# SoyeonHH/MMDA

Hardware: AMD Instinct MI355X
Metric: training samples/sec on MOSEI-shaped synthetic batch (higher is better)
Workload: dtype bf16; 1 GPU; MISA train step, MOSEI shapes B=32/GPU T=50 (d_t,d_v,d_a)=(300,35,74) hidden=128 V=20000, bf16 MFMA operands fp32 accumulate, dropout on, full lengths; global_batch=32, seq_len=50, parallelism=single, use_confidNet=False, rnncell=lstm, dp_global_stats=False

## Files before the change

### mmda_amd/csrc/fused_rows.h

```cpp
#pragma once
#include "../../include/mmda_hip.h"
#include <stdint.h>

struct FusedBwdC {
  int B, hs, ncls, nb;
  const float* tcp; const float* scores; const float* d_tcp; const float* d_scores; float* d_logits;
  float p_cls; uint64_t seed; int site_cls;
  const float* head_w;
  float* d_hfused;
  mmda_ln_bwd_args ln2;
  float* pg_parts;
  const float* d_recon; const float* rec_wT; float* rec_part;
};

struct FusedBwdA {
  int B, hs, nhead, nb;
  mmda_ln_bwd_args ln1;
  const float* ffn_parts; int n_parts; float* d_x1;
  const float* d_attn_out; const float* out_wT; float* d_ctx;
  const float* qkv; const float* probs; float* d_qkv; float p_tf; uint64_t seed; int site_attn;
  const float* in_wT;
  const float* d_recon;
  const float* rec_part;
  const float* rec_wT;
  const float* x6;
  float* d_x6;
  const float* priv_wT;
  const float* sh_wT;
  float* d_orig;
  mmda_ln_bwd_args lnp[3];
  float* pg_parts;
  unsigned long long* dbg;
  const unsigned* wait_flag; unsigned wait_value; unsigned* wait_err;
};

struct FusedFwdA {
  int B, hs, nhead, nb;
  const float* x6;
  const float* rec_w; const float* rec_b; float* recon;
  const float* in_w; const float* in_b; float* qkv;
  float* ctx; float* probs; float p_tf; uint64_t seed; int site_attn;
  const float* out_w; const float* out_b; float* attn_out;
  mmda_ln_args ln1;
  const float* orig; float* d_recon; float* d_orig; float recon_inv_n, recon_scale;
  int split_recon;
};
struct FusedFwdC {
  int B, hs, ncls, nb;
  mmda_ln_args ln2;
  const float* ffn_parts; int n_parts; const float* b2; float* f2;
  const float* hfused; const float* head_w; const float* head_b; float* logits;
  float threshold; float* tcp; float* scores; float* labels; float p_cls; uint64_t seed; int site_cls;
  const float* emo; float* d_scores;
};
struct FusedFfnFwd {
  int M, hs, F, S;
  const float* x1; const float* w1; const float* b1; float* f1;
  float p; uint64_t seed; int site;
  const float* w2;
  float* parts;
};
struct FusedFfnBwd {
  int M, hs, F, S;
  const float* d_f2; const float* f1; float gate_scale;
  const float* l2_wT;
  float* d_f1;
  const float* l1_wT;
  float* parts;
};
int mmda_fused_ffn_fwd(const FusedFfnFwd* a, void* stream);
int mmda_fused_ffn_bwd(const FusedFfnBwd* a, void* stream);
int mmda_fused_fwd_a(const FusedFwdA* a, void* stream);
int mmda_fused_fwd_c(const FusedFwdC* a, void* stream);
int mmda_fused_bwd_c(const FusedBwdC* a, void* stream);
int mmda_fused_bwd_a(const FusedBwdA* a, void* stream);
constexpr int FUSED_PG_SLOTS = 5;
int mmda_fused_pg_finish(const float* pg_parts, int B, int hs, float* const* dgamma, float* const* dbeta, void* stream);
extern "C" int mmda_debug_set_fused_stamps(void* device_buffer);
```

### mmda_amd/csrc/fused_rows.hip

```cpp
#include "common.h"
#include "rowlocal.h"
#include "fused_rows.h"

namespace {

typedef __attribute__((ext_vector_type(4))) float f4;
constexpr int FR_THREADS = 512;

struct MacRound { f4 a[8], b[8]; };
constexpr int WL_LD = 128 + 4;
struct WRows { f4 g[8]; };
__device__ __forceinline__ void wrows_load(WRows& W, const float* __restrict__ bblk, int ldb, int lane) {
#pragma unroll
  for (int j = 0; j < 8; ++j) W.g[j] = *reinterpret_cast<const f4*>(bblk + (int64_t)(2 * j + (lane >> 5)) * ldb + 4 * (lane & 31));
}
__device__ __forceinline__ void wrows_to_lds(const WRows& W, float* wl, int lane) {
#pragma unroll
  for (int j = 0; j < 8; ++j) *reinterpret_cast<f4*>(wl + (2 * j + (lane >> 5)) * WL_LD + 4 * (lane & 31)) = W.g[j];
}
__device__ __forceinline__ void mac_frags(MacRound& R, const float* arow , const float* wl, int lane) {
  const int r16 = lane & 15, g = lane >> 4;
  const f4 z = {0.f, 0.f, 0.f, 0.f};
#pragma unroll
  for (int c = 0; c < 8; ++c) {
    R.a[c] = arow ? *reinterpret_cast<const f4*>(arow + 16 * c + 4 * g) : z;
    R.b[c] = *reinterpret_cast<const f4*>(wl + r16 * WL_LD + 16 * c + 4 * g);
  }
}
__device__ __forceinline__ void mac_run(f32x4& acc, const MacRound& R) {
#pragma unroll
  for (int c = 0; c < 8; ++c)
#pragma unroll
    for (int s = 0; s < 4; ++s) acc = __builtin_amdgcn_mfma_f32_16x16x4f32(R.a[c][s], R.b[c][s], acc, 0, 0, 0);
}
template <int NR>
__device__ __forceinline__ void tile_mac_chain(f32x4& acc, const float* const (&ar)[NR], const float* const (&bblk)[NR], const int (&ldb)[NR],
                                               int lane, float* wl ) {
  WRows W;
  MacRound R;
  wrows_load(W, bblk[0], ldb[0], lane);
#pragma unroll
  for (int r = 0; r < NR; ++r) {
    wrows_to_lds(W, wl, lane);
    if (r + 1 < NR) wrows_load(W, bblk[r + 1], ldb[r + 1], lane);
    mac_frags(R, ar[r], wl, lane);
    mac_run(acc, R);
  }
}

__device__ __forceinline__ float sum_parts(const float* __restrict__ p, int n, int64_t stride) {
  float acc = 0.f;
  int q = 0;
  for (; q + 16 <= n; q += 16) {
    float v[16];
#pragma unroll
    for (int u = 0; u < 16; ++u) v[u] = p[(q + u) * stride];
#pragma unroll
    for (int u = 0; u < 16; ++u) acc += v[u];
  }
  for (; q < n; ++q) acc += p[q * stride];
  return acc;
}

template <typename RowOff, typename Finish>
__device__ __forceinline__ void sum_parts_rows(const float* __restrict__ parts, int n, int64_t stride, int groups, RowOff row_off, f4* lds,
                                               Finish finish) {
  const int n0 = (n + 1) >> 1;
  for (int it = threadIdx.x; it < 2 * groups; it += FR_THREADS) {
    const int gi = it % groups, half = it / groups;
    const float* p = parts + row_off(gi) + (int64_t)(half ? n0 : 0) * stride;
    const int cnt = half ? n - n0 : n0;
    f4 acc = {0.f, 0.f, 0.f, 0.f};
    int q = 0;
    for (; q + 16 <= cnt; q += 16) {
      f4 v[16];
#pragma unroll
      for (int u = 0; u < 16; ++u) v[u] = *reinterpret_cast<const f4*>(p + (q + u) * stride);
#pragma unroll
      for (int u = 0; u < 16; ++u) acc += v[u];
    }
    for (; q < cnt; ++q) acc += *reinterpret_cast<const f4*>(p + q * stride);
    lds[half * groups + gi] = acc;
  }
  __syncthreads();
  for (int gi = threadIdx.x; gi < groups; gi += FR_THREADS) finish(gi, lds[gi] + lds[groups + gi]);
  __syncthreads();
}

__device__ __forceinline__ void stage_sync() {
  __threadfence_block();
  __syncthreads();
}

constexpr int LDS_A_FLOATS = 12 * (384 + 4) + 18 * (128 + 4);
template <typename SrcOf>
__device__ __forceinline__ void stage_rows(float* lds, int nrows, int K, SrcOf src_of) {
  const int per_row = K >> 2;
  for (int e = threadIdx.x; e < nrows * per_row; e += FR_THREADS) {
    const int r = e / per_row, c = e % per_row;
    const float* src = src_of(r);
    const f4 z = {0.f, 0.f, 0.f, 0.f};
    *reinterpret_cast<f4*>(lds + r * (K + 4) + 4 * c) = src ? *reinterpret_cast<const f4*>(src + 4 * c) : z;
  }
  __syncthreads();
}

template <typename RowOf>
__device__ __forceinline__ void ln_bwd_rows(const mmda_ln_bwd_args& a, int nrows, RowOf row_of, float* red ,
                                            float* part) {
  const int lane = threadIdx.x & 63, wave = threadIdx.x >> 6;
  float dg[2] = {0.f, 0.f}, db[2] = {0.f, 0.f};
  for (int i = wave; i < nrows; i += FR_THREADS / 64) ln_bwd_row<2>(a, row_of(i), lane, dg, db);
  if (part == nullptr) return;
#pragma unroll
  for (int q = 0; q < 2; ++q) { red[(0 * 8 + wave) * 128 + q * 64 + lane] = dg[q]; red[(1 * 8 + wave) * 128 + q * 64 + lane] = db[q]; }
  __syncthreads();
  for (int i = threadIdx.x; i < 128; i += FR_THREADS) {
    float gsum = 0.f, bsum = 0.f;
#pragma unroll
    for (int w = 0; w < 8; ++w) { gsum += red[(0 * 8 + w) * 128 + i]; bsum += red[(1 * 8 + w) * 128 + i]; }
    part[i] = i < a.n ? gsum : 0.f;
    part[128 + i] = i < a.n ? bsum : 0.f;
  }
  __syncthreads();
}
__device__ __forceinline__ float* pg_slot(float* parts, int b, int k) { return parts ? parts + ((int64_t)b * FUSED_PG_SLOTS + k) * 256 : nullptr; }
__device__ __forceinline__ void pg_zero_rest(float* parts, int b0, int nb, int k) {
  if (!parts) return;
  for (int e = threadIdx.x; e < (nb - 1) * 256; e += FR_THREADS) pg_slot(parts, b0 + 1 + e / 256, k)[e % 256] = 0.f;
}

__device__ __forceinline__ void rec_part_rows(const FusedBwdC& P, int b0, int nb, float* lds_a, float* lds_w) {
  const int B = P.B, hs = P.hs;
  const int lane = threadIdx.x & 63, wave = threadIdx.x >> 6;
  const int r16 = lane & 15, g = lane >> 4;
  const int nmod = 3 * nb;
  const bool mok = r16 < nmod;
  const int mi = mok ? r16 / nb : 0;
  const int col = wave * 16 + r16;
  stage_rows(lds_a, nmod, hs, [&](int r) { return P.d_recon + ((int64_t)(r / nb) * B + b0 + (r % nb)) * hs; });
  f32x4 acc = {0.f, 0.f, 0.f, 0.f};
  const float* row = mok ? lds_a + r16 * (hs + 4) : nullptr;
  const float* const ar[3] = {(mok && mi == 0) ? row : nullptr, (mok && mi == 1) ? row : nullptr, (mok && mi == 2) ? row : nullptr};
  const float* rw = P.rec_wT + (int64_t)wave * 16 * hs;
  const float* const bb[3] = {rw, rw + (int64_t)hs * hs, rw + (int64_t)2 * hs * hs};
  const int ld[3] = {hs, hs, hs};
  tile_mac_chain<3>(acc, ar, bb, ld, lane, lds_w + wave * 16 * WL_LD);
#pragma unroll
  for (int i = 0; i < 4; ++i) {
    const int r = 4 * g + i;
    if (r < nmod) P.rec_part[((int64_t)(r / nb) * B + b0 + (r % nb)) * hs + col] = acc[i];
  }
}

__global__ __launch_bounds__(FR_THREADS) void fused_bwd_c_kernel(FusedBwdC P) {
  __shared__ float red[2 * 8 * 128];
  __shared__ __attribute__((aligned(16))) float lds_a[6 * (128 + 4)];
  __shared__ __attribute__((aligned(16))) float lds_w[8 * 16 * WL_LD];
  const int nblk = (P.B + P.nb - 1) / P.nb;
  if ((int)blockIdx.x >= nblk) {
    const int rb0 = ((int)blockIdx.x - nblk) * P.nb;
    rec_part_rows(P, rb0, min(P.nb, P.B - rb0), lds_a, lds_w);
    return;
  }
  const int b0 = (int)blockIdx.x * P.nb;
  const int nb = min(P.nb, P.B - b0);
  const int NC = 6 + P.ncls, B = P.B, hs = P.hs;
  for (int e = threadIdx.x; e < nb * NC; e += FR_THREADS) {
    const int b = b0 + e / NC, c = e % NC;
    float g = 0.f;
    if (c < 6) {
      if (P.d_tcp) { const float t = P.tcp[b * 6 + c]; g = P.d_tcp[b * 6 + c] * t * (1.f - t); }
    } else {
      const int k = c - 6;
      if (P.d_scores) {
        const float s = P.scores[b * P.ncls + k];
        g = P.d_scores[b * P.ncls + k] * s * (1.f - s) * drop_mul(P.p_cls, P.seed, P.site_cls, (uint64_t)(b * P.ncls + k));
      }
    }
    P.d_logits[b * NC + c] = g;
  }
  stage_sync();
  const int W6 = 6 * hs;
  for (int e = threadIdx.x; e < nb * W6; e += FR_THREADS) {
    const int b = b0 + e / W6, n = e % W6;
    float acc = 0.f;
    for (int c = 0; c < NC; ++c) acc += P.d_logits[b * NC + c] * P.head_w[(int64_t)c * W6 + n];
    P.d_hfused[(int64_t)b * W6 + n] = acc;
  }
  stage_sync();
  ln_bwd_rows(P.ln2, S6K * nb, [&](int i) { return (i / nb) * B + b0 + (i % nb); }, red, pg_slot(P.pg_parts, b0, 0));
  pg_zero_rest(P.pg_parts, b0, nb, 0);
}

__global__ __launch_bounds__(FR_THREADS) void fused_bwd_a_kernel(FusedBwdA P) {
  __shared__ float red[2 * 8 * 128];
  __shared__ __attribute__((aligned(16))) float lds_a[LDS_A_FLOATS];
  __shared__ __attribute__((aligned(16))) float lds_w[8 * 16 * WL_LD];
  const int b0 = (int)blockIdx.x * P.nb;
  const int nb = min(P.nb, P.B - b0);
  const int B = P.B, hs = P.hs;
  const int lane = threadIdx.x & 63, wave = threadIdx.x >> 6;
  const int r16 = lane & 15, g = lane >> 4;
  const int64_t BH = (int64_t)B * hs;
  int stamp_i = 0;
  auto stamp = [&]() { if (P.dbg && blockIdx.x == 0 && threadIdx.x == 0) P.dbg[stamp_i] = __builtin_readcyclecounter(); ++stamp_i; };
  stamp();
  flag_wait(P.wait_flag, P.wait_value, P.wait_err);
  if (P.ffn_parts) {
    const int64_t MH = (int64_t)S6K * B * hs;
    auto off = [&](int gi) { const int i = gi / (hs / 4); return ((int64_t)(i / nb) * B + b0 + (i % nb)) * hs + 4 * (gi % (hs / 4)); };
    sum_parts_rows(P.ffn_parts, P.n_parts, MH, S6K * nb * (hs / 4), off, reinterpret_cast<f4*>(lds_a), [&](int gi, f4 t) {
      f4* d = reinterpret_cast<f4*>(P.d_x1 + off(gi));
      *d = *d + t;
    });
    stage_sync();
  }
  ln_bwd_rows(P.ln1, S6K * nb, [&](int i) { return (i / nb) * B + b0 + (i % nb); }, red, pg_slot(P.pg_parts, b0, 1));
  pg_zero_rest(P.pg_parts, b0, nb, 1);
  stage_sync();
  stamp();
  const int ntok = S6K * nb;
  const bool rok = r16 < ntok;
  const int tj = rok ? r16 / nb : 0;
  const int col = wave * 16 + r16;
  {
    f32x4 acc = {0.f, 0.f, 0.f, 0.f};
    stage_rows(lds_a, ntok, hs, [&](int r) { return P.d_attn_out + ((int64_t)(r / nb) * B + b0 + (r % nb)) * hs; });
    const float* const ar[1] = {rok ? lds_a + r16 * (hs + 4) : nullptr};
    const float* const bb[1] = {P.out_wT + (int64_t)wave * 16 * hs};
    const int ld[1] = {hs};
    tile_mac_chain<1>(acc, ar, bb, ld, lane, lds_w + wave * 16 * WL_LD);
#pragma unroll
    for (int i = 0; i < 4; ++i) {
      const int r = 4 * g + i;
      if (r < ntok) P.d_ctx[((int64_t)(r / nb) * B + b0 + (r % nb)) * hs + col] = acc[i];
    }
  }
  stage_sync();
  stamp();
  for (int pr = wave; pr < nb * P.nhead; pr += FR_THREADS / 64)
    attn_bwd_hd64_one(P.qkv, P.probs, P.d_ctx, B, P.d_qkv, P.p_tf, P.seed, P.site_attn, P.nhead, (b0 + pr / P.nhead) * P.nhead + pr % P.nhead, lane);
  stage_sync();
  stamp();
  {
    f32x4 acc = {0.f, 0.f, 0.f, 0.f};
    float* lds_r = lds_a + 12 * (3 * hs + 4);
    stage_rows(lds_a, ntok, 3 * hs, [&](int r) { return P.d_qkv + ((int64_t)(r / nb) * B + b0 + (r % nb)) * 3 * hs; });
    const float* qrow = rok ? lds_a + r16 * (3 * hs + 4) : nullptr;
    const float* wrow = P.in_wT + (int64_t)wave * 16 * 3 * hs;
    if (P.rec_part) {
      const float* const ar[3] = {qrow, qrow ? qrow + 128 : nullptr, qrow ? qrow + 256 : nullptr};
      const float* const bb[3] = {wrow, wrow + 128, wrow + 256};
      const int ld[3] = {3 * hs, 3 * hs, 3 * hs};
      tile_mac_chain<3>(acc, ar, bb, ld, lane, lds_w + wave * 16 * WL_LD);
    } else {
      stage_rows(lds_r, ntok, hs, [&](int r) { return P.d_recon + ((int64_t)((r / nb) % 3) * B + b0 + (r % nb)) * hs; });
      const float* rec_row = rok ? lds_r + r16 * (hs + 4) : nullptr;
      const float* const ar[6] = {qrow, qrow ? qrow + 128 : nullptr, qrow ? qrow + 256 : nullptr, (rok && tj % 3 == 0) ? rec_row : nullptr,
                                  (rok && tj % 3 == 1) ? rec_row : nullptr, (rok && tj % 3 == 2) ? rec_row : nullptr};
      const float* recw = P.rec_wT + (int64_t)wave * 16 * hs;
      const float* const bb[6] = {wrow, wrow + 128, wrow + 256, recw, recw + (int64_t)hs * hs, recw + (int64_t)2 * hs * hs};
      const int ld[6] = {3 * hs, 3 * hs, 3 * hs, hs, hs, hs};
      tile_mac_chain<6>(acc, ar, bb, ld, lane, lds_w + wave * 16 * WL_LD);
    }
#pragma unroll
    for (int i = 0; i < 4; ++i) {
      const int r = 4 * g + i;
      if (r < ntok) {
        const int64_t o = ((int64_t)(r / nb) * B + b0 + (r % nb)) * hs + col;
        const float s = P.x6[o];
        float t = acc[i];
        if (P.rec_part) t += P.rec_part[((int64_t)((r / nb) % 3) * B + b0 + (r % nb)) * hs + col];
        P.d_x6[o] = (P.d_x6[o] + t) * (s * (1.f - s));
      }
    }
  }
  stage_sync();
  stamp();
  const int nmod = 3 * nb;
  const bool mok = r16 < nmod;
  const int mi = mok ? r16 / nb : 0;
  {
    f32x4 acc = {0.f, 0.f, 0.f, 0.f};
    stage_rows(lds_a, 2 * nmod, hs, [&](int r) { return P.d_x6 + ((int64_t)((r / nmod) * 3 + (r % nmod) / nb) * B + b0 + (r % nb)) * hs; });
    const float* prow = mok ? lds_a + r16 * (hs + 4) : nullptr;
    const float* const ar[4] = {mok ? lds_a + (nmod + r16) * (hs + 4) : nullptr, (mok && mi == 0) ? prow : nullptr,
                                (mok && mi == 1) ? prow : nullptr, (mok && mi == 2) ? prow : nullptr};
    const float* pw = P.priv_wT + (int64_t)wave * 16 * hs;
    const float* const bb[4] = {P.sh_wT + (int64_t)wave * 16 * hs, pw, pw + (int64_t)hs * hs, pw + (int64_t)2 * hs * hs};
    const int ld[4] = {hs, hs, hs, hs};
    tile_mac_chain<4>(acc, ar, bb, ld, lane, lds_w + wave * 16 * WL_LD);
#pragma unroll
    for (int i = 0; i < 4; ++i) {
      const int r = 4 * g + i;
      if (r < nmod) {
        const int64_t o = ((int64_t)(r / nb) * B + b0 + (r % nb)) * hs + col;
        P.d_orig[o] += acc[i];
      }
    }
  }
  stage_sync();
  stamp();
  for (int i = wave; i < 3 * nb; i += FR_THREADS / 64) {
    const mmda_ln_bwd_args& a = P.lnp[i / nb];
    float dg[2] = {0.f, 0.f}, db[2] = {0.f, 0.f};
    ln_bwd_row<2>(a, b0 + i % nb, lane, dg, db);
    float* part = pg_slot(P.pg_parts, b0 + i % nb, 2 + i / nb);
    if (part) {
#pragma unroll
      for (int q = 0; q < 2; ++q) {
        const int c = q * 64 + lane;
        part[c] = c < a.n ? dg[q] : 0.f;
        part[128 + c] = c < a.n ? db[q] : 0.f;
      }
    }
  }
  (void)BH;
  stamp();
}

__global__ __launch_bounds__(FR_THREADS) void fused_fwd_a_kernel(FusedFwdA P) {
  __shared__ __attribute__((aligned(16))) float lds_a[LDS_A_FLOATS];
  __shared__ __attribute__((aligned(16))) float lds_w[8 * 16 * WL_LD];
  const int nblk = (P.B + P.nb - 1) / P.nb;
  const bool do_recon = !P.split_recon || (int)blockIdx.x >= nblk;
  const bool do_chain = !P.split_recon || (int)blockIdx.x < nblk;
  const int b0 = ((int)blockIdx.x % nblk) * P.nb;
  const int nb = min(P.nb, P.B - b0);
  const int B = P.B, hs = P.hs;
  const int lane = threadIdx.x & 63, wave = threadIdx.x >> 6;
  const int r16 = lane & 15, g = lane >> 4;
  const int ntok = S6K * nb, nmod = 3 * nb;
  const bool rok = r16 < ntok;
  const bool mok = r16 < nmod;
  const int mi = mok ? r16 / nb : 0;
  const int col = wave * 16 + r16;
  stage_rows(lds_a, ntok, hs, [&](int r) { return P.x6 + ((int64_t)(r / nb) * B + b0 + (r % nb)) * hs; });
  if (do_recon) {
  for (int e = threadIdx.x; e < nmod * (hs / 4); e += FR_THREADS) {
    const int r = e / (hs / 4), c = e % (hs / 4);
    const f4 a = *reinterpret_cast<const f4*>(lds_a + r * (hs + 4) + 4 * c), b2 = *reinterpret_cast<const f4*>(lds_a + (nmod + r) * (hs + 4) + 4 * c);
    *reinterpret_cast<f4*>(lds_a + (12 + r) * (hs + 4) + 4 * c) = a + b2;
  }
  __syncthreads();
  {
    f32x4 acc = {0.f, 0.f, 0.f, 0.f};
    const float* srow = mok ? lds_a + (12 + r16) * (hs + 4) : nullptr;
    const float* const ar[3] = {(mok && mi == 0) ? srow : nullptr, (mok && mi == 1) ? srow : nullptr, (mok && mi == 2) ? srow : nullptr};
    const float* rw = P.rec_w + (int64_t)wave * 16 * hs;
    const float* const bb[3] = {rw, rw + (int64_t)hs * hs, rw + (int64_t)2 * hs * hs};
    const int ld[3] = {hs, hs, hs};
    tile_mac_chain<3>(acc, ar, bb, ld, lane, lds_w + wave * 16 * WL_LD);
#pragma unroll
    for (int i = 0; i < 4; ++i) {
      const int r = 4 * g + i;
      if (r < nmod) {
        const int64_t o = ((int64_t)(r / nb) * B + b0 + (r % nb)) * hs + col;
        const float rv = acc[i] + P.rec_b[(r / nb) * hs + col];
        P.recon[o] = rv;
        if (P.d_recon) {
          const float d = rv - P.orig[o];
          const float gr = 2.f * d * P.recon_inv_n * P.recon_scale;
          P.d_recon[o] = gr;
          P.d_orig[o] = 0.f - gr;
        }
      }
    }
  }
  }
  if (!do_chain) return;
#pragma unroll 1
  for (int pass = 0; pass < 3; ++pass) {
    const int n = pass * 128 + col;
    f32x4 acc = {0.f, 0.f, 0.f, 0.f};
    const float* const ar[1] = {rok ? lds_a + r16 * (hs + 4) : nullptr};
    const float* const bb[1] = {P.in_w + (int64_t)(pass * 128 + wave * 16) * hs};
    const int ld[1] = {hs};
    tile_mac_chain<1>(acc, ar, bb, ld, lane, lds_w + wave * 16 * WL_LD);
    const float bias = P.in_b[n];
#pragma unroll
    for (int i = 0; i < 4; ++i) {
      const int r = 4 * g + i;
      if (r < ntok) P.qkv[((int64_t)(r / nb) * B + b0 + (r % nb)) * 3 * hs + n] = acc[i] + bias;
    }
  }
  stage_sync();
  for (int pr = wave; pr < nb * P.nhead; pr += FR_THREADS / 64)
    attn_fwd_hd64_one(P.qkv, B, P.ctx, P.probs, P.p_tf, P.seed, P.site_attn, P.nhead, (b0 + pr / P.nhead) * P.nhead + pr % P.nhead, lane);
  stage_sync();
  {
    f32x4 acc = {0.f, 0.f, 0.f, 0.f};
    stage_rows(lds_a, ntok, hs, [&](int r) { return P.ctx + ((int64_t)(r / nb) * B + b0 + (r % nb)) * hs; });
    const float* const ar[1] = {rok ? lds_a + r16 * (hs + 4) : nullptr};
    const float* const bb[1] = {P.out_w + (int64_t)wave * 16 * hs};
    const int ld[1] = {hs};
    tile_mac_chain<1>(acc, ar, bb, ld, lane, lds_w + wave * 16 * WL_LD);
    const float bias = P.out_b[col];
#pragma unroll
    for (int i = 0; i < 4; ++i) {
      const int r = 4 * g + i;
      if (r < ntok) P.attn_out[((int64_t)(r / nb) * B + b0 + (r % nb)) * hs + col] = acc[i] + bias;
    }
  }
  stage_sync();
  for (int i = wave; i < ntok; i += FR_THREADS / 64) ln_fwd_row<2>(P.ln1, (i / nb) * B + b0 + (i % nb), lane);
}

__global__ __launch_bounds__(FR_THREADS) void fused_fwd_c_kernel(FusedFwdC P) {
  __shared__ f4 sp[2 * 12 * 32];
  const int b0 = (int)blockIdx.x * P.nb;
  const int nb = min(P.nb, P.B - b0);
  const int B = P.B, hs = P.hs, NC = 6 + P.ncls, W6 = 6 * hs;
  const int lane = threadIdx.x & 63, wave = threadIdx.x >> 6;
  if (P.ffn_parts) {
    const int64_t MH = (int64_t)S6K * B * hs;
    auto off = [&](int gi) { const int i = gi / (hs / 4); return ((int64_t)(i / nb) * B + b0 + (i % nb)) * hs + 4 * (gi % (hs / 4)); };
    sum_parts_rows(P.ffn_parts, P.n_parts, MH, S6K * nb * (hs / 4), off, sp, [&](int gi, f4 t) {
      const float* b = P.b2 + 4 * (gi % (hs / 4));
      *reinterpret_cast<f4*>(P.f2 + off(gi)) = t + f4{b[0], b[1], b[2], b[3]};
    });
    stage_sync();
  }
  for (int i = wave; i < S6K * nb; i += FR_THREADS / 64) ln_fwd_row<2>(P.ln2, (i / nb) * B + b0 + (i % nb), lane);
  stage_sync();
  for (int e = wave; e < nb * NC; e += FR_THREADS / 64) {
    const int b = b0 + e / NC, c = e % NC;
    const float* x = P.hfused + (int64_t)b * W6;
    const float* w = P.head_w + (int64_t)c * W6;
    float acc = 0.f;
    for (int k = lane * 4; k < W6; k += 256) {
      const f4 xv = *reinterpret_cast<const f4*>(x + k), wv = *reinterpret_cast<const f4*>(w + k);
      acc += xv[0] * wv[0] + xv[1] * wv[1] + xv[2] * wv[2] + xv[3] * wv[3];
    }
    acc = wave_sum(acc);
    if (lane == 0) {
      const float z = acc + P.head_b[c];
      P.logits[b * NC + c] = z;
      if (c < 6) {
        P.tcp[b * 6 + c] = sigmoidf_(z);
      } else {
        const int k = c - 6;
        const float sc = sigmoidf_(z * drop_mul(P.p_cls, P.seed, P.site_cls, (uint64_t)(b * P.ncls + k)));
        P.scores[b * P.ncls + k] = sc;
        P.labels[b * P.ncls + k] = sc > P.threshold ? 1.f : 0.f;
        if (P.d_scores) {
          const float yv = P.emo[b * P.ncls + k];
          P.d_scores[b * P.ncls + k] = (sc - yv) / fmaxf(sc * (1.f - sc), 1e-12f) / B;
        }
      }
    }
  }
}

constexpr int FFN_RB = 48, FFN_S = 32;
constexpr int FFN_LDS_X = FFN_RB * (128 + 4), FFN_LDS_H = FFN_RB * (FFN_S + 4);

struct FfnGeom { int rb0, nrows, j; };

template <typename Epi1, typename Store2>
__device__ __forceinline__ void ffn_two_products(const float* xs, float* hs_, const float* __restrict__ b1rows ,
                                                 int ldb1, const float* __restrict__ b2rows , int ldb2,
                                                 Epi1 epi1, Store2 store2) {
  const int lane = threadIdx.x & 63, wave = threadIdx.x >> 6;
  const int r16 = lane & 15, g = lane >> 4;
  {
    const int ct = wave >> 2;
    f4 bw[8];
    const float* brow = b1rows + (int64_t)(ct * 16 + r16) * ldb1;
#pragma unroll
    for (int c = 0; c < 8; ++c) bw[c] = *reinterpret_cast<const f4*>(brow + 16 * c + 4 * g);
#pragma unroll
    for (int q = 0; q < (FFN_RB / 16 + 3) / 4; ++q) {
      const int rt = (wave & 3) + 4 * q;
      if (rt >= FFN_RB / 16) break;
      const float* arow = xs + (rt * 16 + r16) * (128 + 4);
      f32x4 acc = {0.f, 0.f, 0.f, 0.f};
#pragma unroll
      for (int c = 0; c < 8; ++c) {
        const f4 a = *reinterpret_cast<const f4*>(arow + 16 * c + 4 * g);
#pragma unroll
        for (int s = 0; s < 4; ++s) acc = __builtin_amdgcn_mfma_f32_16x16x4f32(a[s], bw[c][s], acc, 0, 0, 0);
      }
#pragma unroll
      for (int i = 0; i < 4; ++i) {
        const int row = rt * 16 + 4 * g + i, unit = ct * 16 + r16;
        hs_[row * (FFN_S + 4) + unit] = epi1(row, unit, acc[i]);
      }
    }
  }
  __syncthreads();
  {
    f4 bw[2];
    const float* brow = b2rows + (int64_t)(wave * 16 + r16) * ldb2;
#pragma unroll
    for (int c = 0; c < 2; ++c) bw[c] = *reinterpret_cast<const f4*>(brow + 16 * c + 4 * g);
#pragma unroll
    for (int rt = 0; rt < FFN_RB / 16; ++rt) {
      const float* arow = hs_ + (rt * 16 + r16) * (FFN_S + 4);
      f32x4 acc = {0.f, 0.f, 0.f, 0.f};
#pragma unroll
      for (int c = 0; c < 2; ++c) {
        const f4 a = *reinterpret_cast<const f4*>(arow + 16 * c + 4 * g);
#pragma unroll
        for (int s = 0; s < 4; ++s) acc = __builtin_amdgcn_mfma_f32_16x16x4f32(a[s], bw[c][s], acc, 0, 0, 0);
      }
#pragma unroll
      for (int i = 0; i < 4; ++i) store2(rt * 16 + 4 * g + i, wave * 16 + r16, acc[i]);
    }
  }
}

__device__ __forceinline__ void ffn_stage_x(float* xs, const float* __restrict__ X, int rb0, int M) {
  constexpr int PER = FFN_RB * 32 / FR_THREADS;
  f4 v[PER];
#pragma unroll
  for (int u = 0; u < PER; ++u) {
    const int e = threadIdx.x + u * FR_THREADS, r = e >> 5, c = e & 31;
    v[u] = *reinterpret_cast<const f4*>(X + (int64_t)min(rb0 + r, M - 1) * 128 + 4 * c);
  }
#pragma unroll
  for (int u = 0; u < PER; ++u) {
    const int e = threadIdx.x + u * FR_THREADS, r = e >> 5, c = e & 31;
    const f4 z = {0.f, 0.f, 0.f, 0.f};
    *reinterpret_cast<f4*>(xs + r * (128 + 4) + 4 * c) = (rb0 + r < M) ? v[u] : z;
  }
  __syncthreads();
}

__global__ __launch_bounds__(FR_THREADS) void fused_ffn_fwd_kernel(FusedFfnFwd P) {
  extern __shared__ __attribute__((aligned(16))) float ffn_lds[];
  float* xs = ffn_lds; float* hs_ = ffn_lds + FFN_LDS_X;
  const int nsl = P.F / FFN_S;
  const int j = (int)blockIdx.x % nsl, rb0 = ((int)blockIdx.x / nsl) * FFN_RB;
  ffn_stage_x(xs, P.x1, rb0, P.M);
  float* part = P.parts + (int64_t)j * P.M * P.hs;
  ffn_two_products(xs, hs_, P.w1 + (int64_t)j * FFN_S * P.hs, P.hs, P.w2 + (int64_t)j * FFN_S, P.F,
    [&](int row, int unit, float v) {
      const int m = rb0 + row, n = j * FFN_S + unit;
      v += P.b1[n];
      v = fmaxf(v, 0.f);
      if (P.p > 0.f) v *= drop_mul(P.p, P.seed, P.site, (uint64_t)m * P.F + n);
      if (m < P.M) P.f1[(int64_t)m * P.F + n] = v; else v = 0.f;
      return v;
    },
    [&](int row, int col, float v) { if (rb0 + row < P.M) part[(int64_t)(rb0 + row) * P.hs + col] = v; });
}

__global__ __launch_bounds__(FR_THREADS) void fused_ffn_bwd_kernel(FusedFfnBwd P) {
  extern __shared__ __attribute__((aligned(16))) float ffn_lds[];
  float* xs = ffn_lds; float* hs_ = ffn_lds + FFN_LDS_X;
  const int nsl = P.F / FFN_S;
  const int j = (int)blockIdx.x % nsl, rb0 = ((int)blockIdx.x / nsl) * FFN_RB;
  ffn_stage_x(xs, P.d_f2, rb0, P.M);
  float* part = P.parts + (int64_t)j * P.M * P.hs;
  ffn_two_products(xs, hs_, P.l2_wT + (int64_t)j * FFN_S * P.hs, P.hs, P.l1_wT + (int64_t)j * FFN_S, P.F,
    [&](int row, int unit, float v) {
      const int m = rb0 + row, n = j * FFN_S + unit;
      if (m >= P.M) return 0.f;
      v *= (P.f1[(int64_t)m * P.F + n] > 0.f) ? P.gate_scale : 0.f;
      P.d_f1[(int64_t)m * P.F + n] = v;
      return v;
    },
    [&](int row, int col, float v) { if (rb0 + row < P.M) part[(int64_t)(rb0 + row) * P.hs + col] = v; });
}

}

int mmda_fused_ffn_fwd(const FusedFfnFwd* a, void* stream) {
  if (!a || a->M <= 0 || a->hs != 128 || a->S != FFN_S || a->F <= 0 || (a->F % FFN_S)) return MMDA_EINVAL;
  const int lds = (FFN_LDS_X + FFN_LDS_H) * 4;
  static bool attr = false;
  if (!attr) { (void)hipFuncSetAttribute(reinterpret_cast<const void*>(fused_ffn_fwd_kernel), hipFuncAttributeMaxDynamicSharedMemorySize, lds); attr = true; }
  hipLaunchKernelGGL(fused_ffn_fwd_kernel, dim3((a->F / FFN_S) * ceil_div(a->M, FFN_RB)), dim3(FR_THREADS), lds, (hipStream_t)stream, *a);
  MMDA_CHECK_LAUNCH("mmda_fused_ffn_fwd");
  return MMDA_OK;
}

int mmda_fused_ffn_bwd(const FusedFfnBwd* a, void* stream) {
  if (!a || a->M <= 0 || a->hs != 128 || a->S != FFN_S || a->F <= 0 || (a->F % FFN_S)) return MMDA_EINVAL;
  const int lds = (FFN_LDS_X + FFN_LDS_H) * 4;
  static bool attr = false;
  if (!attr) { (void)hipFuncSetAttribute(reinterpret_cast<const void*>(fused_ffn_bwd_kernel), hipFuncAttributeMaxDynamicSharedMemorySize, lds); attr = true; }
  hipLaunchKernelGGL(fused_ffn_bwd_kernel, dim3((a->F / FFN_S) * ceil_div(a->M, FFN_RB)), dim3(FR_THREADS), lds, (hipStream_t)stream, *a);
  MMDA_CHECK_LAUNCH("mmda_fused_ffn_bwd");
  return MMDA_OK;
}

int mmda_fused_fwd_a(const FusedFwdA* a, void* stream) {
  if (!a || a->B <= 0 || a->nb <= 0 || a->nb > 2 || a->hs != 128 || a->nhead != 2 || a->ln1.n != 128) return MMDA_EINVAL;
  if (a->d_recon && (!a->orig || !a->d_orig)) return MMDA_EINVAL;
  static const int split_on = mmda_env_int("MMDA_FUSED_SPLIT", 1);
  FusedFwdA f = *a;
  const int nblk = ceil_div(a->B, a->nb);
  f.split_recon = (split_on && nblk <= 64) ? 1 : 0;
  hipLaunchKernelGGL(fused_fwd_a_kernel, dim3(f.split_recon ? 2 * nblk : nblk), dim3(FR_THREADS), 0, (hipStream_t)stream, f);
  MMDA_CHECK_LAUNCH("mmda_fused_fwd_a");
  return MMDA_OK;
}

int mmda_fused_fwd_c(const FusedFwdC* a, void* stream) {
  if (!a || a->B <= 0 || a->nb <= 0 || a->nb > 2 || a->hs != 128 || a->ln2.n != 128 || (a->d_scores && !a->emo)) return MMDA_EINVAL;
  hipLaunchKernelGGL(fused_fwd_c_kernel, dim3(ceil_div(a->B, a->nb)), dim3(FR_THREADS), 0, (hipStream_t)stream, *a);
  MMDA_CHECK_LAUNCH("mmda_fused_fwd_c");
  return MMDA_OK;
}

struct FusedPgOut { float* dgamma[FUSED_PG_SLOTS]; float* dbeta[FUSED_PG_SLOTS]; };
__global__ __launch_bounds__(256) void fused_pg_finish_kernel(const float* __restrict__ parts, int B, int hs, FusedPgOut out) {
  __shared__ float sub[256];
  const int e = blockIdx.x * 16 + (threadIdx.x >> 4);
  const int j = threadIdx.x & 15;
  const bool ok = e < FUSED_PG_SLOTS * 256;
  const int k = ok ? e / 256 : 0, which = (e % 256) / 128, c = e % 128;
  const float* p = parts + (int64_t)k * 256 + which * 128 + c;
  float acc = 0.f;
  if (ok) {
    const int64_t st = (int64_t)FUSED_PG_SLOTS * 256;
    int b = j;
    for (; b + 7 * 16 < B; b += 8 * 16) {
      float v[8];
#pragma unroll
      for (int u = 0; u < 8; ++u) v[u] = p[(b + 16 * u) * st];
#pragma unroll
      for (int u = 0; u < 8; ++u) acc += v[u];
    }
    for (; b < B; b += 16) acc += p[b * st];
  }
  sub[threadIdx.x] = acc;
  __syncthreads();
  float* dst = which ? out.dbeta[k] : out.dgamma[k];
  if (ok && j == 0 && dst && c < hs) {
    float t = 0.f;
#pragma unroll
    for (int u = 0; u < 16; ++u) t += sub[(threadIdx.x & ~15) + u];
    dst[c] += t;
  }
}

int mmda_fused_pg_finish(const float* pg_parts, int B, int hs, float* const* dgamma, float* const* dbeta, void* stream) {
  if (!pg_parts || B <= 0 || hs != 128 || !dgamma || !dbeta) return MMDA_EINVAL;
  FusedPgOut out;
  for (int k = 0; k < FUSED_PG_SLOTS; ++k) { out.dgamma[k] = dgamma[k]; out.dbeta[k] = dbeta[k]; }
  hipLaunchKernelGGL(fused_pg_finish_kernel, dim3(FUSED_PG_SLOTS * 256 / 16), dim3(256), 0, (hipStream_t)stream, pg_parts, B, hs, out);
  MMDA_CHECK_LAUNCH("mmda_fused_pg_finish");
  return MMDA_OK;
}

int mmda_fused_bwd_c(const FusedBwdC* a, void* stream) {
  if (!a || a->B <= 0 || a->nb <= 0 || a->hs != 128 || a->ln2.n != 128) return MMDA_EINVAL;
  if ((a->ln2.dgamma || a->ln2.dbeta) && !a->pg_parts) return MMDA_EINVAL;
  if (a->rec_part && (!a->d_recon || !a->rec_wT || a->nb > 2)) return MMDA_EINVAL;
  hipLaunchKernelGGL(fused_bwd_c_kernel, dim3(ceil_div(a->B, a->nb) * (a->rec_part ? 2 : 1)), dim3(FR_THREADS), 0, (hipStream_t)stream, *a);
  MMDA_CHECK_LAUNCH("mmda_fused_bwd_c");
  return MMDA_OK;
}

static unsigned long long* g_fr_dbg = nullptr;
extern "C" int mmda_debug_set_fused_stamps(void* device_buffer) { g_fr_dbg = (unsigned long long*)device_buffer; return MMDA_OK; }

int mmda_fused_bwd_a(const FusedBwdA* a, void* stream) {
  if (!a || a->B <= 0 || a->nb <= 0 || a->nb > 2 || a->hs != 128 || a->nhead != 2) return MMDA_EINVAL;
  if ((a->ln1.dgamma || a->ln1.dbeta || a->lnp[0].dgamma || a->lnp[0].dbeta) && !a->pg_parts) return MMDA_EINVAL;
  FusedBwdA P = *a;
  P.dbg = g_fr_dbg;
  hipLaunchKernelGGL(fused_bwd_a_kernel, dim3(ceil_div(a->B, a->nb)), dim3(FR_THREADS), 0, (hipStream_t)stream, P);
  MMDA_CHECK_LAUNCH("mmda_fused_bwd_a");
  return MMDA_OK;
}
```

### mmda_amd/csrc/rowlocal.h

```cpp
#pragma once
#include "common.h"

namespace {

__device__ __forceinline__ int64_t perm_row(int row, int S, int Bp) {
  if (S <= 0) return row;
  int s = row / Bp, b = row % Bp;
  return (int64_t)b * S + s;
}

template <int NQ>
__device__ __forceinline__ void ln_bwd_row(const mmda_ln_bwd_args& a, int row, int lane, float (&dg)[NQ], float (&db)[NQ]) {
  const int n = a.n;
  const float mean = a.mean[row], rstd = a.rstd[row];
  const int64_t drow = perm_row(row, a.permute_S, a.permute_B);
  float xh[NQ], gdy[NQ];
  float s1 = 0.f, s2 = 0.f;
#pragma unroll
  for (int q = 0; q < NQ; ++q) {
    int i = lane + 64 * q;
    xh[q] = 0.f; gdy[q] = 0.f;
    if (i < n) {
      int64_t idx = (int64_t)row * n + i;
      float x = act_fwd_p(a.act, a.x[idx], a.actp, (uint64_t)idx);
      if (a.res) x += a.res[idx] * drop_mul(a.drop_p, a.drop_seed, a.drop_site, (uint64_t)idx);
      float dy = a.dy[drow * n + i];
      xh[q] = (x - mean) * rstd;
      gdy[q] = dy * a.gamma[i];
      dg[q] += dy * xh[q];
      db[q] += dy;
      s1 += gdy[q];
      s2 += gdy[q] * xh[q];
    }
  }
  s1 = wave_sum(s1) / n;
  s2 = wave_sum(s2) / n;
  float dslope = 0.f;
#pragma unroll
  for (int q = 0; q < NQ; ++q) {
    int i = lane + 64 * q;
    if (i < n) {
      int64_t idx = (int64_t)row * n + i;
      float dxp = rstd * (gdy[q] - s1 - xh[q] * s2);
      if (a.d_x) {
        const float z = a.x[idx];
        float d = dxp * act_bwd_p(a.act, z, a.actp, (uint64_t)idx);
        a.d_x[idx] = a.accumulate_dx ? a.d_x[idx] + d : d;
        if (a.act == MMDA_ACT_PRELU && z <= 0.f) dslope += dxp * z;
      }
      if (a.d_res) a.d_res[idx] = dxp * drop_mul(a.drop_p, a.drop_seed, a.drop_site, (uint64_t)idx);
    }
  }
  if (a.act == MMDA_ACT_PRELU && a.d_x && a.actp.dslope) {
    dslope = wave_sum(dslope);
    if (lane == 0) atomicAdd(a.actp.dslope, dslope);
  }
}

template <int NQ>
__device__ __forceinline__ void ln_fwd_row(const mmda_ln_args& a, int row, int lane) {
  const int n = a.n;
  float v[NQ];
  float s = 0.f;
#pragma unroll
  for (int q = 0; q < NQ; ++q) {
    int i = lane + 64 * q;
    float x = 0.f;
    if (i < n) {
      int64_t idx = (int64_t)row * n + i;
      x = act_fwd_p(a.act, a.x[idx], a.actp, (uint64_t)idx);
      if (a.res) x += a.res[idx] * drop_mul(a.drop_p, a.drop_seed, a.drop_site, (uint64_t)idx);
    }
    v[q] = x;
    s += x;
  }
  const float mean = wave_sum(s) / n;
  float ss = 0.f;
#pragma unroll
  for (int q = 0; q < NQ; ++q) {
    int i = lane + 64 * q;
    float d = (i < n) ? v[q] - mean : 0.f;
    ss += d * d;
  }
  const float var = wave_sum(ss) / n;
  const float rstd = 1.0f / sqrtf(var + a.eps);
  if (lane == 0) {
    if (a.mean) a.mean[row] = mean;
    if (a.rstd) a.rstd[row] = rstd;
  }
  const int64_t orow = perm_row(row, a.permute_S, a.permute_B);
#pragma unroll
  for (int q = 0; q < NQ; ++q) {
    int i = lane + 64 * q;
    float y = 0.f;
    if (i < n) { y = (v[q] - mean) * rstd * a.gamma[i] + a.beta[i]; if (a.y) a.y[orow * n + i] = y; }
    if (a.y_bf16 && i < a.ld_bf16) reinterpret_cast<unsigned short*>(a.y_bf16)[orow * a.ld_bf16 + i] = f2bf(y);
  }
}

constexpr int S6K = 6;

__device__ __forceinline__ void attn_fwd_hd64_one(const float* __restrict__ qkv, int B, float* ctx, float* probs, float p, uint64_t seed,
                                                  int site, int nhead, int bh, int d) {
  constexpr int S = S6K, hd = 64;
  const int E = hd * nhead;
  const int b = bh / nhead, h = bh % nhead;
  float q[S], k[S], v[S];
#pragma unroll
  for (int s = 0; s < S; ++s) {
    const float* row = qkv + ((int64_t)s * B + b) * 3 * E + h * hd + d;
    q[s] = row[0]; k[s] = row[E]; v[s] = row[2 * E];
  }
  const float scale = 1.0f / sqrtf((float)hd);
  float pr[S][S];
#pragma unroll
  for (int i = 0; i < S; ++i)
#pragma unroll
    for (int j = 0; j < S; ++j) pr[i][j] = wave_sum(q[i] * k[j]) * scale;
#pragma unroll
  for (int i = 0; i < S; ++i) {
    float m = -INFINITY;
#pragma unroll
    for (int j = 0; j < S; ++j) m = fmaxf(m, pr[i][j]);
    float sum = 0.f;
#pragma unroll
    for (int j = 0; j < S; ++j) { pr[i][j] = expf(pr[i][j] - m); sum += pr[i][j]; }
    const float inv = 1.0f / sum;
#pragma unroll
    for (int j = 0; j < S; ++j) {
      const float pv = pr[i][j] * inv;
      const int64_t pi = ((int64_t)bh * S + i) * S + j;
      if (d == 0) probs[pi] = pv;
      pr[i][j] = pv * drop_mul(p, seed, site, (uint64_t)pi);
    }
  }
#pragma unroll
  for (int s = 0; s < S; ++s) {
    float acc = 0.f;
#pragma unroll
    for (int j = 0; j < S; ++j) acc += pr[s][j] * v[j];
    ctx[((int64_t)s * B + b) * E + h * hd + d] = acc;
  }
}


__device__ __forceinline__ void attn_bwd_hd64_one(const float* __restrict__ qkv, const float* __restrict__ probs, const float* __restrict__ dctx,
                                                  int B, float* dqkv, float p, uint64_t seed, int site, int nhead, int bh, int d) {
  constexpr int S = S6K, hd = 64;
  const int E = hd * nhead;
  const int b = bh / nhead, h = bh % nhead;
  float q[S], k[S], v[S], dc[S];
#pragma unroll
  for (int s = 0; s < S; ++s) {
    const float* row = qkv + ((int64_t)s * B + b) * 3 * E + h * hd + d;
    q[s] = row[0]; k[s] = row[E]; v[s] = row[2 * E];
    dc[s] = dctx[((int64_t)s * B + b) * E + h * hd + d];
  }
  float P[S][S], Pd[S][S], dS[S][S];
#pragma unroll
  for (int i = 0; i < S; ++i)
#pragma unroll
    for (int j = 0; j < S; ++j) {
      const int64_t pi = (int64_t)bh * S * S + i * S + j;
      const float mul = drop_mul(p, seed, site, (uint64_t)pi);
      P[i][j] = probs[pi];
      Pd[i][j] = P[i][j] * mul;
      dS[i][j] = wave_sum(dc[i] * v[j]) * mul;
    }
#pragma unroll
  for (int i = 0; i < S; ++i) {
    float dot = 0.f;
#pragma unroll
    for (int j = 0; j < S; ++j) dot += dS[i][j] * P[i][j];
#pragma unroll
    for (int j = 0; j < S; ++j) dS[i][j] = P[i][j] * (dS[i][j] - dot);
  }
  const float scale = 1.0f / sqrtf((float)hd);
#pragma unroll
  for (int s = 0; s < S; ++s) {
    float dq = 0.f, dk = 0.f, dv = 0.f;
#pragma unroll
    for (int j = 0; j < S; ++j) {
      dq += dS[s][j] * k[j];
      dk += dS[j][s] * q[j];
      dv += Pd[j][s] * dc[j];
    }
    float* row = dqkv + ((int64_t)s * B + b) * 3 * E + h * hd + d;
    row[0] = dq * scale; row[E] = dk * scale; row[2 * E] = dv;
  }
}

}
```

Before: 53290 samples/s.

## Keep fused-kernel stage intermediates in LDS and prefetch weight tiles across stages

The fused forward/backward row kernels now write each stage's results to dedicated LDS regions and read them there in the next stage (LN backward dy/dres, d_ctx, d_qkv, d_x6, d_orig, attention qkv/ctx). This replaces global-memory round trips and the stage_rows restaging, and drops several fence+sync pairs. Weight-tile loads get a deeper lookahead and are started early so they overlap the previous stage, with the next stage's first tile prefetched inside the MAC chain. The changes also preload head weights into registers, add debug stamps to the forward kernel, and add host-side argument checks that enforce the aliasing assumptions the LDS reuse depends on. In exchange, LDS use and register pressure go up, and correctness now relies on those aliasing checks.

```diff
diff --git a/mmda_amd/csrc/fused_rows.h b/mmda_amd/csrc/fused_rows.h
--- a/mmda_amd/csrc/fused_rows.h
+++ b/mmda_amd/csrc/fused_rows.h
@@ -44,6 +44,7 @@
   mmda_ln_args ln1;
   const float* orig; float* d_recon; float* d_orig; float recon_inv_n, recon_scale;
   int split_recon;
+  unsigned long long* dbg;
 };
 struct FusedFwdC {
   int B, hs, ncls, nb;
diff --git a/mmda_amd/csrc/fused_rows.hip b/mmda_amd/csrc/fused_rows.hip
--- a/mmda_amd/csrc/fused_rows.hip
+++ b/mmda_amd/csrc/fused_rows.hip
@@ -33,16 +33,24 @@
 #pragma unroll
     for (int s = 0; s < 4; ++s) acc = __builtin_amdgcn_mfma_f32_16x16x4f32(R.a[c][s], R.b[c][s], acc, 0, 0, 0);
 }
+#ifndef FR_LOOK
+#define FR_LOOK 2
+#endif
 template <int NR>
-__device__ __forceinline__ void tile_mac_chain(f32x4& acc, const float* const (&ar)[NR], const float* const (&bblk)[NR], const int (&ldb)[NR],
-                                               int lane, float* wl ) {
-  WRows W;
+__device__ __forceinline__ void tile_mac_chain_pre(f32x4& acc, WRows& W, const float* const (&ar)[NR], const float* const (&bblk)[NR],
+                                                   const int (&ldb)[NR], int lane, float* wl ,
+                                                   const float* next_blk = nullptr, int next_ld = 0) {
+  constexpr int LA = FR_LOOK < NR ? FR_LOOK : (NR > 1 ? NR - 1 : 1);
+  WRows Q[LA];
   MacRound R;
-  wrows_load(W, bblk[0], ldb[0], lane);
+  Q[0] = W;
+#pragma unroll
+  for (int r = 1; r < LA; ++r) wrows_load(Q[r], bblk[r], ldb[r], lane);
 #pragma unroll
   for (int r = 0; r < NR; ++r) {
-    wrows_to_lds(W, wl, lane);
-    if (r + 1 < NR) wrows_load(W, bblk[r + 1], ldb[r + 1], lane);
+    wrows_to_lds(Q[r % LA], wl, lane);
+    if (r + LA < NR) wrows_load(Q[r % LA], bblk[r + LA], ldb[r + LA], lane);
+    else if (r == (NR > LA ? NR - LA : 0) && next_blk) wrows_load(W, next_blk, next_ld, lane);
     mac_frags(R, ar[r], wl, lane);
     mac_run(acc, R);
   }
@@ -92,7 +100,11 @@
   __syncthreads();
 }
 
-constexpr int LDS_A_FLOATS = 12 * (384 + 4) + 18 * (128 + 4);
+constexpr int LD1 = 128 + 4, LD3 = 384 + 4;
+constexpr int FWD_S = 12 * LD1, FWD_Q = FWD_S + 6 * LD1, FWD_C = FWD_Q + 12 * LD3, FWD_LDS_FLOATS = FWD_C + 12 * LD1;
+constexpr int BWD_R = 12 * LD3, BWD_D1 = 3072, BWD_A = BWD_D1 + 12 * LD1, BWD_C = BWD_R + 18 * LD1, BWD_X = BWD_C + 12 * LD1,
+              BWD_O = BWD_X + 12 * LD1, BWD_LDS_FLOATS = BWD_O + 6 * LD1;
+static_assert(BWD_A + 12 * LD1 <= BWD_C, "the early regions lie under Q + R");
 template <typename SrcOf>
 __device__ __forceinline__ void stage_rows(float* lds, int nrows, int K, SrcOf src_of) {
   const int per_row = K >> 2;
@@ -107,10 +119,11 @@
 
 template <typename RowOf>
 __device__ __forceinline__ void ln_bwd_rows(const mmda_ln_bwd_args& a, int nrows, RowOf row_of, float* red ,
-                                            float* part) {
+                                            float* part, const float* lds_dy = nullptr, float* lds_dres = nullptr) {
   const int lane = threadIdx.x & 63, wave = threadIdx.x >> 6;
   float dg[2] = {0.f, 0.f}, db[2] = {0.f, 0.f};
-  for (int i = wave; i < nrows; i += FR_THREADS / 64) ln_bwd_row<2>(a, row_of(i), lane, dg, db);
+  for (int i = wave; i < nrows; i += FR_THREADS / 64)
+    ln_bwd_row<2>(a, row_of(i), lane, dg, db, lds_dy ? lds_dy + i * LD1 : nullptr, lds_dres ? lds_dres + i * LD1 : nullptr);
   if (part == nullptr) return;
 #pragma unroll
   for (int q = 0; q < 2; ++q) { red[(0 * 8 + wave) * 128 + q * 64 + lane] = dg[q]; red[(1 * 8 + wave) * 128 + q * 64 + lane] = db[q]; }
@@ -138,14 +151,16 @@
   const bool mok = r16 < nmod;
   const int mi = mok ? r16 / nb : 0;
   const int col = wave * 16 + r16;
+  const float* rw = P.rec_wT + (int64_t)wave * 16 * hs;
+  WRows W;
+  wrows_load(W, rw, hs, lane);
   stage_rows(lds_a, nmod, hs, [&](int r) { return P.d_recon + ((int64_t)(r / nb) * B + b0 + (r % nb)) * hs; });
   f32x4 acc = {0.f, 0.f, 0.f, 0.f};
   const float* row = mok ? lds_a + r16 * (hs + 4) : nullptr;
   const float* const ar[3] = {(mok && mi == 0) ? row : nullptr, (mok && mi == 1) ? row : nullptr, (mok && mi == 2) ? row : nullptr};
-  const float* rw = P.rec_wT + (int64_t)wave * 16 * hs;
   const float* const bb[3] = {rw, rw + (int64_t)hs * hs, rw + (int64_t)2 * hs * hs};
   const int ld[3] = {hs, hs, hs};
-  tile_mac_chain<3>(acc, ar, bb, ld, lane, lds_w + wave * 16 * WL_LD);
+  tile_mac_chain_pre<3>(acc, W, ar, bb, ld, lane, lds_w + wave * 16 * WL_LD);
 #pragma unroll
   for (int i = 0; i < 4; ++i) {
     const int r = 4 * g + i;
@@ -166,6 +181,18 @@
   const int b0 = (int)blockIdx.x * P.nb;
   const int nb = min(P.nb, P.B - b0);
   const int NC = 6 + P.ncls, B = P.B, hs = P.hs;
+  const int W6 = 6 * hs;
+  constexpr int HP = 2, HC = 16;
+  float hw[HP][HC];
+#pragma unroll
+  for (int u = 0; u < HP; ++u) {
+    const int e = threadIdx.x + u * FR_THREADS;
+    const int n = (e < nb * W6 ? e : 0) % W6;
+#pragma unroll
+    for (int c = 0; c < HC; ++c) hw[u][c] = c < NC ? P.head_w[(int64_t)c * W6 + n] : 0.f;
+  }
+  float* lds_l = red;
+  float* lds_h = lds_w;
   for (int e = threadIdx.x; e < nb * NC; e += FR_THREADS) {
     const int b = b0 + e / NC, c = e % NC;
     float g = 0.f;
@@ -179,44 +206,63 @@
       }
     }
     P.d_logits[b * NC + c] = g;
-  }
-  stage_sync();
-  const int W6 = 6 * hs;
-  for (int e = threadIdx.x; e < nb * W6; e += FR_THREADS) {
-    const int b = b0 + e / W6, n = e % W6;
+    lds_l[e] = g;
+  }
+  __syncthreads();
+  auto elem = [&](int e, const float (*pre)[HC] ) {
+    const int sb = e / W6, n = e % W6;
+    const float* dl = lds_l + sb * NC;
     float acc = 0.f;
-    for (int c = 0; c < NC; ++c) acc += P.d_logits[b * NC + c] * P.head_w[(int64_t)c * W6 + n];
-    P.d_hfused[(int64_t)b * W6 + n] = acc;
-  }
-  stage_sync();
-  ln_bwd_rows(P.ln2, S6K * nb, [&](int i) { return (i / nb) * B + b0 + (i % nb); }, red, pg_slot(P.pg_parts, b0, 0));
+    int c = 0;
+    if (pre) {
+#pragma unroll
+      for (int q = 0; q < HC; ++q)
+        if (q < NC) acc += dl[q] * (*pre)[q];
+      c = HC;
+    }
+    for (; c < NC; ++c) acc += dl[c] * P.head_w[(int64_t)c * W6 + n];
+    P.d_hfused[(int64_t)(b0 + sb) * W6 + n] = acc;
+    lds_h[((n / hs) * nb + sb) * LD1 + n % hs] = acc;
+  };
+#pragma unroll
+  for (int u = 0; u < HP; ++u)
+    if ((int)threadIdx.x + u * FR_THREADS < nb * W6) elem(threadIdx.x + u * FR_THREADS, &hw[u]);
+  for (int e = threadIdx.x + HP * FR_THREADS; e < nb * W6; e += FR_THREADS) elem(e, nullptr);
+  __syncthreads();
+  ln_bwd_rows(P.ln2, S6K * nb, [&](int i) { return (i / nb) * B + b0 + (i % nb); }, red, pg_slot(P.pg_parts, b0, 0), lds_h);
   pg_zero_rest(P.pg_parts, b0, nb, 0);
 }
 
 __global__ __launch_bounds__(FR_THREADS) void fused_bwd_a_kernel(FusedBwdA P) {
   __shared__ float red[2 * 8 * 128];
-  __shared__ __attribute__((aligned(16))) float lds_a[LDS_A_FLOATS];
+  __shared__ __attribute__((aligned(16))) float lds_a[BWD_LDS_FLOATS];
   __shared__ __attribute__((aligned(16))) float lds_w[8 * 16 * WL_LD];
   const int b0 = (int)blockIdx.x * P.nb;
   const int nb = min(P.nb, P.B - b0);
   const int B = P.B, hs = P.hs;
   const int lane = threadIdx.x & 63, wave = threadIdx.x >> 6;
   const int r16 = lane & 15, g = lane >> 4;
-  const int64_t BH = (int64_t)B * hs;
+  float* wl = lds_w + wave * 16 * WL_LD;
+  float* lds_d1 = lds_a + BWD_D1; float* lds_da = lds_a + BWD_A; float* lds_c = lds_a + BWD_C; float* lds_x = lds_a + BWD_X;
+  float* lds_o = lds_a + BWD_O;
   int stamp_i = 0;
   auto stamp = [&]() { if (P.dbg && blockIdx.x == 0 && threadIdx.x == 0) P.dbg[stamp_i] = __builtin_readcyclecounter(); ++stamp_i; };
   stamp();
+  WRows W;
+  wrows_load(W, P.out_wT + (int64_t)wave * 16 * hs, hs, lane);
   flag_wait(P.wait_flag, P.wait_value, P.wait_err);
   if (P.ffn_parts) {
     const int64_t MH = (int64_t)S6K * B * hs;
     auto off = [&](int gi) { const int i = gi / (hs / 4); return ((int64_t)(i / nb) * B + b0 + (i % nb)) * hs + 4 * (gi % (hs / 4)); };
     sum_parts_rows(P.ffn_parts, P.n_parts, MH, S6K * nb * (hs / 4), off, reinterpret_cast<f4*>(lds_a), [&](int gi, f4 t) {
       f4* d = reinterpret_cast<f4*>(P.d_x1 + off(gi));
-      *d = *d + t;
+      const f4 v = *d + t;
+      *d = v;
+      *reinterpret_cast<f4*>(lds_d1 + (gi / (hs / 4)) * LD1 + 4 * (gi % (hs / 4))) = v;
     });
-    stage_sync();
-  }
-  ln_bwd_rows(P.ln1, S6K * nb, [&](int i) { return (i / nb) * B + b0 + (i % nb); }, red, pg_slot(P.pg_parts, b0, 1));
+  }
+  ln_bwd_rows(P.ln1, S6K * nb, [&](int i) { return (i / nb) * B + b0 + (i % nb); }, red, pg_slot(P.pg_parts, b0, 1),
+              P.ffn_parts ? lds_d1 : nullptr, lds_da);
   pg_zero_rest(P.pg_parts, b0, nb, 1);
   stage_sync();
   stamp();
@@ -224,88 +270,114 @@
   const bool rok = r16 < ntok;
   const int tj = rok ? r16 / nb : 0;
   const int col = wave * 16 + r16;
+  const float* wrow = P.in_wT + (int64_t)wave * 16 * 3 * hs;
   {
     f32x4 acc = {0.f, 0.f, 0.f, 0.f};
-    stage_rows(lds_a, ntok, hs, [&](int r) { return P.d_attn_out + ((int64_t)(r / nb) * B + b0 + (r % nb)) * hs; });
-    const float* const ar[1] = {rok ? lds_a + r16 * (hs + 4) : nullptr};
+    const float* const ar[1] = {rok ? lds_da + r16 * LD1 : nullptr};
     const float* const bb[1] = {P.out_wT + (int64_t)wave * 16 * hs};
     const int ld[1] = {hs};
-    tile_mac_chain<1>(acc, ar, bb, ld, lane, lds_w + wave * 16 * WL_LD);
+    tile_mac_chain_pre<1>(acc, W, ar, bb, ld, lane, wl, wrow, 3 * hs);
 #pragma unroll
     for (int i = 0; i < 4; ++i) {
       const int r = 4 * g + i;
-      if (r < ntok) P.d_ctx[((int64_t)(r / nb) * B + b0 + (r % nb)) * hs + col] = acc[i];
-    }
-  }
-  stage_sync();
-  stamp();
-  for (int pr = wave; pr < nb * P.nhead; pr += FR_THREADS / 64)
-    attn_bwd_hd64_one(P.qkv, P.probs, P.d_ctx, B, P.d_qkv, P.p_tf, P.seed, P.site_attn, P.nhead, (b0 + pr / P.nhead) * P.nhead + pr % P.nhead, lane);
-  stage_sync();
+      if (r < ntok) {
+        P.d_ctx[((int64_t)(r / nb) * B + b0 + (r % nb)) * hs + col] = acc[i];
+        lds_c[r * LD1 + col] = acc[i];
+      }
+    }
+  }
+  __syncthreads();
+  stamp();
+  for (int pr = wave; pr < nb * P.nhead; pr += FR_THREADS / 64) {
+    const int sb = pr / P.nhead;
+    attn_bwd_hd64_one(P.qkv, P.probs, P.d_ctx, B, P.d_qkv, P.p_tf, P.seed, P.site_attn, P.nhead, (b0 + sb) * P.nhead + pr % P.nhead, lane,
+                      lds_c + sb * LD1, nb * LD1, lds_a + sb * LD3, nb * LD3);
+  }
+  __syncthreads();
   stamp();
   {
     f32x4 acc = {0.f, 0.f, 0.f, 0.f};
-    float* lds_r = lds_a + 12 * (3 * hs + 4);
-    stage_rows(lds_a, ntok, 3 * hs, [&](int r) { return P.d_qkv + ((int64_t)(r / nb) * B + b0 + (r % nb)) * 3 * hs; });
-    const float* qrow = rok ? lds_a + r16 * (3 * hs + 4) : nullptr;
-    const float* wrow = P.in_wT + (int64_t)wave * 16 * 3 * hs;
+    float* lds_r = lds_a + BWD_R;
+    float e_s[4], e_d[4], e_p[4];
+#pragma unroll
+    for (int i = 0; i < 4; ++i) {
+      const int r = 4 * g + i;
+      e_s[i] = e_d[i] = e_p[i] = 0.f;
+      if (r < ntok) {
+        const int64_t o = ((int64_t)(r / nb) * B + b0 + (r % nb)) * hs + col;
+        e_s[i] = P.x6[o];
+        e_d[i] = P.d_x6[o];
+        if (P.rec_part) e_p[i] = P.rec_part[((int64_t)((r / nb) % 3) * B + b0 + (r % nb)) * hs + col];
+      }
+    }
+    const float* qrow = rok ? lds_a + r16 * LD3 : nullptr;
+    const float* shw = P.sh_wT + (int64_t)wave * 16 * hs;
     if (P.rec_part) {
       const float* const ar[3] = {qrow, qrow ? qrow + 128 : nullptr, qrow ? qrow + 256 : nullptr};
       const float* const bb[3] = {wrow, wrow + 128, wrow + 256};
       const int ld[3] = {3 * hs, 3 * hs, 3 * hs};
-      tile_mac_chain<3>(acc, ar, bb, ld, lane, lds_w + wave * 16 * WL_LD);
+      tile_mac_chain_pre<3>(acc, W, ar, bb, ld, lane, wl, shw, hs);
     } else {
       stage_rows(lds_r, ntok, hs, [&](int r) { return P.d_recon + ((int64_t)((r / nb) % 3) * B + b0 + (r % nb)) * hs; });
-      const float* rec_row = rok ? lds_r + r16 * (hs + 4) : nullptr;
+      const float* rec_row = rok ? lds_r + r16 * LD1 : nullptr;
       const float* const ar[6] = {qrow, qrow ? qrow + 128 : nullptr, qrow ? qrow + 256 : nullptr, (rok && tj % 3 == 0) ? rec_row : nullptr,
                                   (rok && tj % 3 == 1) ? rec_row : nullptr, (rok && tj % 3 == 2) ? rec_row : nullptr};
       const float* recw = P.rec_wT + (int64_t)wave * 16 * hs;
       const float* const bb[6] = {wrow, wrow + 128, wrow + 256, recw, recw + (int64_t)hs * hs, recw + (int64_t)2 * hs * hs};
       const int ld[6] = {3 * hs, 3 * hs, 3 * hs, hs, hs, hs};
-      tile_mac_chain<6>(acc, ar, bb, ld, lane, lds_w + wave * 16 * WL_LD);
+      tile_mac_chain_pre<6>(acc, W, ar, bb, ld, lane, wl, shw, hs);
     }
 #pragma unroll
     for (int i = 0; i < 4; ++i) {
       const int r = 4 * g + i;
       if (r < ntok) {
         const int64_t o = ((int64_t)(r / nb) * B + b0 + (r % nb)) * hs + col;
-        const float s = P.x6[o];
+        const float s = e_s[i];
         float t = acc[i];
-        if (P.rec_part) t += P.rec_part[((int64_t)((r / nb) % 3) * B + b0 + (r % nb)) * hs + col];
-        P.d_x6[o] = (P.d_x6[o] + t) * (s * (1.f - s));
-      }
-    }
-  }
-  stage_sync();
+        if (P.rec_part) t += e_p[i];
+        const float v = (e_d[i] + t) * (s * (1.f - s));
+        P.d_x6[o] = v;
+        lds_x[r * LD1 + col] = v;
+      }
+    }
+  }
+  __syncthreads();
   stamp();
   const int nmod = 3 * nb;
   const bool mok = r16 < nmod;
   const int mi = mok ? r16 / nb : 0;
   {
     f32x4 acc = {0.f, 0.f, 0.f, 0.f};
-    stage_rows(lds_a, 2 * nmod, hs, [&](int r) { return P.d_x6 + ((int64_t)((r / nmod) * 3 + (r % nmod) / nb) * B + b0 + (r % nb)) * hs; });
-    const float* prow = mok ? lds_a + r16 * (hs + 4) : nullptr;
-    const float* const ar[4] = {mok ? lds_a + (nmod + r16) * (hs + 4) : nullptr, (mok && mi == 0) ? prow : nullptr,
+    float e_o[4];
+#pragma unroll
+    for (int i = 0; i < 4; ++i) {
+      const int r = 4 * g + i;
+      e_o[i] = r < nmod ? P.d_orig[((int64_t)(r / nb) * B + b0 + (r % nb)) * hs + col] : 0.f;
+    }
+    const float* prow = mok ? lds_x + r16 * LD1 : nullptr;
+    const float* const ar[4] = {mok ? lds_x + (nmod + r16) * LD1 : nullptr, (mok && mi == 0) ? prow : nullptr,
                                 (mok && mi == 1) ? prow : nullptr, (mok && mi == 2) ? prow : nullptr};
     const float* pw = P.priv_wT + (int64_t)wave * 16 * hs;
     const float* const bb[4] = {P.sh_wT + (int64_t)wave * 16 * hs, pw, pw + (int64_t)hs * hs, pw + (int64_t)2 * hs * hs};
     const int ld[4] = {hs, hs, hs, hs};
-    tile_mac_chain<4>(acc, ar, bb, ld, lane, lds_w + wave * 16 * WL_LD);
+    tile_mac_chain_pre<4>(acc, W, ar, bb, ld, lane, wl);
 #pragma unroll
     for (int i = 0; i < 4; ++i) {
       const int r = 4 * g + i;
       if (r < nmod) {
         const int64_t o = ((int64_t)(r / nb) * B + b0 + (r % nb)) * hs + col;
-        P.d_orig[o] += acc[i];
-      }
-    }
-  }
-  stage_sync();
+        const float v = e_o[i] + acc[i];
+        P.d_orig[o] = v;
+        lds_o[r * LD1 + col] = v;
+      }
+    }
+  }
+  __syncthreads();
   stamp();
   for (int i = wave; i < 3 * nb; i += FR_THREADS / 64) {
     const mmda_ln_bwd_args& a = P.lnp[i / nb];
     float dg[2] = {0.f, 0.f}, db[2] = {0.f, 0.f};
-    ln_bwd_row<2>(a, b0 + i % nb, lane, dg, db);
+    ln_bwd_row<2>(a, b0 + i % nb, lane, dg, db, lds_o + i * LD1);
     float* part = pg_slot(P.pg_parts, b0 + i % nb, 2 + i / nb);
     if (part) {
 #pragma unroll
@@ -316,12 +388,11 @@
       }
     }
   }
-  (void)BH;
   stamp();
 }
 
 __global__ __launch_bounds__(FR_THREADS) void fused_fwd_a_kernel(FusedFwdA P) {
-  __shared__ __attribute__((aligned(16))) float lds_a[LDS_A_FLOATS];
+  __shared__ __attribute__((aligned(16))) float lds_a[FWD_LDS_FLOATS];
   __shared__ __attribute__((aligned(16))) float lds_w[8 * 16 * WL_LD];
   const int nblk = (P.B + P.nb - 1) / P.nb;
   const bool do_recon = !P.split_recon || (int)blockIdx.x >= nblk;
@@ -336,31 +407,53 @@
   const bool mok = r16 < nmod;
   const int mi = mok ? r16 / nb : 0;
   const int col = wave * 16 + r16;
+  int stamp_i = 8;
+  auto stamp = [&]() { if (P.dbg && blockIdx.x == 0 && threadIdx.x == 0) P.dbg[stamp_i] = __builtin_readcyclecounter(); ++stamp_i; };
+  auto stamp_recon = [&](int i) { if (P.dbg && (int)blockIdx.x == (P.split_recon ? nblk : 0) && threadIdx.x == 0) P.dbg[i] = __builtin_readcyclecounter(); };
+  stamp();
+  float* wl = lds_w + wave * 16 * WL_LD;
+  float* lds_s = lds_a + FWD_S; float* lds_q = lds_a + FWD_Q; float* lds_c = lds_a + FWD_C;
+  float* lds_o = lds_q;
+  const float* inw = P.in_w + (int64_t)wave * 16 * hs;
+  WRows W;
+  wrows_load(W, do_recon ? P.rec_w + (int64_t)wave * 16 * hs : inw, hs, lane);
   stage_rows(lds_a, ntok, hs, [&](int r) { return P.x6 + ((int64_t)(r / nb) * B + b0 + (r % nb)) * hs; });
+  stamp();
   if (do_recon) {
+  stamp_recon(14);
   for (int e = threadIdx.x; e < nmod * (hs / 4); e += FR_THREADS) {
     const int r = e / (hs / 4), c = e % (hs / 4);
-    const f4 a = *reinterpret_cast<const f4*>(lds_a + r * (hs + 4) + 4 * c), b2 = *reinterpret_cast<const f4*>(lds_a + (nmod + r) * (hs + 4) + 4 * c);
-    *reinterpret_cast<f4*>(lds_a + (12 + r) * (hs + 4) + 4 * c) = a + b2;
+    const f4 a = *reinterpret_cast<const f4*>(lds_a + r * LD1 + 4 * c), b2 = *reinterpret_cast<const f4*>(lds_a + (nmod + r) * LD1 + 4 * c);
+    *reinterpret_cast<f4*>(lds_s + r * LD1 + 4 * c) = a + b2;
   }
   __syncthreads();
   {
     f32x4 acc = {0.f, 0.f, 0.f, 0.f};
-    const float* srow = mok ? lds_a + (12 + r16) * (hs + 4) : nullptr;
+    float e_b[4], e_o[4];
+#pragma unroll
+    for (int i = 0; i < 4; ++i) {
+      const int r = 4 * g + i;
+      e_b[i] = e_o[i] = 0.f;
+      if (r < nmod) {
+        e_b[i] = P.rec_b[(r / nb) * hs + col];
+        if (P.d_recon) e_o[i] = P.orig[((int64_t)(r / nb) * B + b0 + (r % nb)) * hs + col];
+      }
+    }
+    const float* srow = mok ? lds_s + r16 * LD1 : nullptr;
     const float* const ar[3] = {(mok && mi == 0) ? srow : nullptr, (mok && mi == 1) ? srow : nullptr, (mok && mi == 2) ? srow : nullptr};
     const float* rw = P.rec_w + (int64_t)wave * 16 * hs;
     const float* const bb[3] = {rw, rw + (int64_t)hs * hs, rw + (int64_t)2 * hs * hs};
     const int ld[3] = {hs, hs, hs};
-    tile_mac_chain<3>(acc, ar, bb, ld, lane, lds_w + wave * 16 * WL_LD);
+    tile_mac_chain_pre<3>(acc, W, ar, bb, ld, lane, wl, do_chain ? inw : nullptr, hs);
 #pragma unroll
     for (int i = 0; i < 4; ++i) {
       const int r = 4 * g + i;
       if (r < nmod) {
         const int64_t o = ((int64_t)(r / nb) * B + b0 + (r % nb)) * hs + col;
-        const float rv = acc[i] + P.rec_b[(r / nb) * hs + col];
+        const float rv = acc[i] + e_b[i];
         P.recon[o] = rv;
         if (P.d_recon) {
-          const float d = rv - P.orig[o];
+          const float d = rv - e_o[i];
           const float gr = 2.f * d * P.recon_inv_n * P.recon_scale;
           P.d_recon[o] = gr;
           P.d_orig[o] = 0.f - gr;
@@ -368,69 +461,109 @@
       }
     }
   }
+  stamp_recon(15);
   }
   if (!do_chain) return;
-#pragma unroll 1
-  for (int pass = 0; pass < 3; ++pass) {
-    const int n = pass * 128 + col;
+  {
+    f32x4 acc[3] = {{0.f, 0.f, 0.f, 0.f}, {0.f, 0.f, 0.f, 0.f}, {0.f, 0.f, 0.f, 0.f}};
+    float bias[3];
+#pragma unroll
+    for (int pass = 0; pass < 3; ++pass) bias[pass] = P.in_b[pass * 128 + col];
+    const float* arow = rok ? lds_a + r16 * LD1 : nullptr;
+    MacRound R;
+#pragma unroll
+    for (int pass = 0; pass < 3; ++pass) {
+      wrows_to_lds(W, wl, lane);
+      if (pass < 2) wrows_load(W, inw + (int64_t)(pass + 1) * 128 * hs, hs, lane);
+      else wrows_load(W, P.out_w + (int64_t)wave * 16 * hs, hs, lane);
+      mac_frags(R, arow, wl, lane);
+      mac_run(acc[pass], R);
+    }
+#pragma unroll
+    for (int pass = 0; pass < 3; ++pass) {
+      const int n = pass * 128 + col;
+#pragma unroll
+      for (int i = 0; i < 4; ++i) {
+        const int r = 4 * g + i;
+        if (r < ntok) {
+          const float v = acc[pass][i] + bias[pass];
+          P.qkv[((int64_t)(r / nb) * B + b0 + (r % nb)) * 3 * hs + n] = v;
+          lds_q[r * LD3 + n] = v;
+        }
+      }
+    }
+  }
+  __syncthreads();
+  stamp();
+  for (int pr = wave; pr < nb * P.nhead; pr += FR_THREADS / 64) {
+    const int sb = pr / P.nhead;
+    attn_fwd_hd64_one(P.qkv, B, P.ctx, P.probs, P.p_tf, P.seed, P.site_attn, P.nhead, (b0 + sb) * P.nhead + pr % P.nhead, lane,
+                      lds_q + sb * LD3, nb * LD3, lds_c + sb * LD1, nb * LD1);
+  }
+  __syncthreads();
+  stamp();
+  {
     f32x4 acc = {0.f, 0.f, 0.f, 0.f};
-    const float* const ar[1] = {rok ? lds_a + r16 * (hs + 4) : nullptr};
-    const float* const bb[1] = {P.in_w + (int64_t)(pass * 128 + wave * 16) * hs};
+    const float bias = P.out_b[col];
+    const float* const ar[1] = {rok ? lds_c + r16 * LD1 : nullptr};
+    const float* const bb[1] = {P.out_w + (int64_t)wave * 16 * hs};
     const int ld[1] = {hs};
-    tile_mac_chain<1>(acc, ar, bb, ld, lane, lds_w + wave * 16 * WL_LD);
-    const float bias = P.in_b[n];
+    tile_mac_chain_pre<1>(acc, W, ar, bb, ld, lane, wl);
 #pragma unroll
     for (int i = 0; i < 4; ++i) {
       const int r = 4 * g + i;
-      if (r < ntok) P.qkv[((int64_t)(r / nb) * B + b0 + (r % nb)) * 3 * hs + n] = acc[i] + bias;
-    }
-  }
-  stage_sync();
-  for (int pr = wave; pr < nb * P.nhead; pr += FR_THREADS / 64)
-    attn_fwd_hd64_one(P.qkv, B, P.ctx, P.probs, P.p_tf, P.seed, P.site_attn, P.nhead, (b0 + pr / P.nhead) * P.nhead + pr % P.nhead, lane);
-  stage_sync();
-  {
-    f32x4 acc = {0.f, 0.f, 0.f, 0.f};
-    stage_rows(lds_a, ntok, hs, [&](int r) { return P.ctx + ((int64_t)(r / nb) * B + b0 + (r % nb)) * hs; });
-    const float* const ar[1] = {rok ? lds_a + r16 * (hs + 4) : nullptr};
-    const float* const bb[1] = {P.out_w + (int64_t)wave * 16 * hs};
-    const int ld[1] = {hs};
-    tile_mac_chain<1>(acc, ar, bb, ld, lane, lds_w + wave * 16 * WL_LD);
-    const float bias = P.out_b[col];
-#pragma unroll
-    for (int i = 0; i < 4; ++i) {
-      const int r = 4 * g + i;
-      if (r < ntok) P.attn_out[((int64_t)(r / nb) * B + b0 + (r % nb)) * hs + col] = acc[i] + bias;
-    }
-  }
-  stage_sync();
-  for (int i = wave; i < ntok; i += FR_THREADS / 64) ln_fwd_row<2>(P.ln1, (i / nb) * B + b0 + (i % nb), lane);
+      if (r < ntok) {
+        const float v = acc[i] + bias;
+        P.attn_out[((int64_t)(r / nb) * B + b0 + (r % nb)) * hs + col] = v;
+        lds_o[r * LD1 + col] = v;
+      }
+    }
+  }
+  __syncthreads();
+  stamp();
+  for (int i = wave; i < ntok; i += FR_THREADS / 64) ln_fwd_row<2>(P.ln1, (i / nb) * B + b0 + (i % nb), lane, lds_a + i * LD1, lds_o + i * LD1);
+  stamp();
 }
 
 __global__ __launch_bounds__(FR_THREADS) void fused_fwd_c_kernel(FusedFwdC P) {
   __shared__ f4 sp[2 * 12 * 32];
+  __shared__ __attribute__((aligned(16))) float lds_f[12 * 128];
+  __shared__ __attribute__((aligned(16))) float lds_h[2 * 6 * 128];
   const int b0 = (int)blockIdx.x * P.nb;
   const int nb = min(P.nb, P.B - b0);
   const int B = P.B, hs = P.hs, NC = 6 + P.ncls, W6 = 6 * hs;
   const int lane = threadIdx.x & 63, wave = threadIdx.x >> 6;
+  constexpr int HP = 2;
+  f4 hw[HP][3];
+#pragma unroll
+  for (int u = 0; u < HP; ++u) {
+    const int e = wave + u * (FR_THREADS / 64);
+    const float* w = P.head_w + (int64_t)((e < nb * NC ? e : 0) % NC) * W6;
+#pragma unroll
+    for (int t = 0; t < 3; ++t) hw[u][t] = *reinterpret_cast<const f4*>(w + lane * 4 + 256 * t);
+  }
   if (P.ffn_parts) {
     const int64_t MH = (int64_t)S6K * B * hs;
     auto off = [&](int gi) { const int i = gi / (hs / 4); return ((int64_t)(i / nb) * B + b0 + (i % nb)) * hs + 4 * (gi % (hs / 4)); };
     sum_parts_rows(P.ffn_parts, P.n_parts, MH, S6K * nb * (hs / 4), off, sp, [&](int gi, f4 t) {
       const float* b = P.b2 + 4 * (gi % (hs / 4));
-      *reinterpret_cast<f4*>(P.f2 + off(gi)) = t + f4{b[0], b[1], b[2], b[3]};
+      const f4 v = t + f4{b[0], b[1], b[2], b[3]};
+      *reinterpret_cast<f4*>(P.f2 + off(gi)) = v;
+      *reinterpret_cast<f4*>(lds_f + 4 * gi) = v;
     });
-    stage_sync();
-  }
-  for (int i = wave; i < S6K * nb; i += FR_THREADS / 64) ln_fwd_row<2>(P.ln2, (i / nb) * B + b0 + (i % nb), lane);
-  stage_sync();
-  for (int e = wave; e < nb * NC; e += FR_THREADS / 64) {
+  }
+  for (int i = wave; i < S6K * nb; i += FR_THREADS / 64)
+    ln_fwd_row<2>(P.ln2, (i / nb) * B + b0 + (i % nb), lane, nullptr, P.ffn_parts ? lds_f + i * 128 : nullptr, lds_h + ((i % nb) * S6K + i / nb) * 128);
+  __syncthreads();
+  auto pair = [&](int e, const f4* pre ) {
     const int b = b0 + e / NC, c = e % NC;
-    const float* x = P.hfused + (int64_t)b * W6;
+    const float* x = lds_h + (e / NC) * W6;
     const float* w = P.head_w + (int64_t)c * W6;
     float acc = 0.f;
-    for (int k = lane * 4; k < W6; k += 256) {
-      const f4 xv = *reinterpret_cast<const f4*>(x + k), wv = *reinterpret_cast<const f4*>(w + k);
+#pragma unroll
+    for (int t = 0; t < 3; ++t) {
+      const int k = lane * 4 + 256 * t;
+      const f4 xv = *reinterpret_cast<const f4*>(x + k), wv = pre ? pre[t] : *reinterpret_cast<const f4*>(w + k);
       acc += xv[0] * wv[0] + xv[1] * wv[1] + xv[2] * wv[2] + xv[3] * wv[3];
     }
     acc = wave_sum(acc);
@@ -450,7 +583,11 @@
         }
       }
     }
-  }
+  };
+#pragma unroll
+  for (int u = 0; u < HP; ++u)
+    if (wave + u * (FR_THREADS / 64) < nb * NC) pair(wave + u * (FR_THREADS / 64), hw[u]);
+  for (int e = wave + HP * (FR_THREADS / 64); e < nb * NC; e += FR_THREADS / 64) pair(e, nullptr);
 }
 
 constexpr int FFN_RB = 48, FFN_S = 32;
@@ -567,6 +704,9 @@
 
 }
 
+static unsigned long long* g_fr_dbg = nullptr;
+extern "C" int mmda_debug_set_fused_stamps(void* device_buffer) { g_fr_dbg = (unsigned long long*)device_buffer; return MMDA_OK; }
+
 int mmda_fused_ffn_fwd(const FusedFfnFwd* a, void* stream) {
   if (!a || a->M <= 0 || a->hs != 128 || a->S != FFN_S || a->F <= 0 || (a->F % FFN_S)) return MMDA_EINVAL;
   const int lds = (FFN_LDS_X + FFN_LDS_H) * 4;
@@ -590,10 +730,12 @@
 int mmda_fused_fwd_a(const FusedFwdA* a, void* stream) {
   if (!a || a->B <= 0 || a->nb <= 0 || a->nb > 2 || a->hs != 128 || a->nhead != 2 || a->ln1.n != 128) return MMDA_EINVAL;
   if (a->d_recon && (!a->orig || !a->d_orig)) return MMDA_EINVAL;
+  if (a->ln1.x != a->x6 || a->ln1.res != a->attn_out || a->ln1.permute_S) return MMDA_EINVAL;
   static const int split_on = mmda_env_int("MMDA_FUSED_SPLIT", 1);
   FusedFwdA f = *a;
   const int nblk = ceil_div(a->B, a->nb);
   f.split_recon = (split_on && nblk <= 64) ? 1 : 0;
+  f.dbg = g_fr_dbg;
   hipLaunchKernelGGL(fused_fwd_a_kernel, dim3(f.split_recon ? 2 * nblk : nblk), dim3(FR_THREADS), 0, (hipStream_t)stream, f);
   MMDA_CHECK_LAUNCH("mmda_fused_fwd_a");
   return MMDA_OK;
@@ -601,6 +743,7 @@
 
 int mmda_fused_fwd_c(const FusedFwdC* a, void* stream) {
   if (!a || a->B <= 0 || a->nb <= 0 || a->nb > 2 || a->hs != 128 || a->ln2.n != 128 || (a->d_scores && !a->emo)) return MMDA_EINVAL;
+  if (a->ln2.y != a->hfused || a->ln2.permute_S != S6K || a->ln2.permute_B != a->B || (a->ffn_parts && a->ln2.res != a->f2)) return MMDA_EINVAL;
   hipLaunchKernelGGL(fused_fwd_c_kernel, dim3(ceil_div(a->B, a->nb)), dim3(FR_THREADS), 0, (hipStream_t)stream, *a);
   MMDA_CHECK_LAUNCH("mmda_fused_fwd_c");
   return MMDA_OK;
@@ -651,17 +794,19 @@
   if (!a || a->B <= 0 || a->nb <= 0 || a->hs != 128 || a->ln2.n != 128) return MMDA_EINVAL;
   if ((a->ln2.dgamma || a->ln2.dbeta) && !a->pg_parts) return MMDA_EINVAL;
   if (a->rec_part && (!a->d_recon || !a->rec_wT || a->nb > 2)) return MMDA_EINVAL;
+  if (a->nb > 2 || a->ncls < 0 || 6 + a->ncls > 64 || a->ln2.dy != a->d_hfused || a->ln2.permute_S != S6K || a->ln2.permute_B != a->B)
+    return MMDA_EINVAL;
   hipLaunchKernelGGL(fused_bwd_c_kernel, dim3(ceil_div(a->B, a->nb) * (a->rec_part ? 2 : 1)), dim3(FR_THREADS), 0, (hipStream_t)stream, *a);
   MMDA_CHECK_LAUNCH("mmda_fused_bwd_c");
   return MMDA_OK;
 }
 
-static unsigned long long* g_fr_dbg = nullptr;
-extern "C" int mmda_debug_set_fused_stamps(void* device_buffer) { g_fr_dbg = (unsigned long long*)device_buffer; return MMDA_OK; }
-
 int mmda_fused_bwd_a(const FusedBwdA* a, void* stream) {
   if (!a || a->B <= 0 || a->nb <= 0 || a->nb > 2 || a->hs != 128 || a->nhead != 2) return MMDA_EINVAL;
   if ((a->ln1.dgamma || a->ln1.dbeta || a->lnp[0].dgamma || a->lnp[0].dbeta) && !a->pg_parts) return MMDA_EINVAL;
+  if (a->ln1.d_res != a->d_attn_out || a->ln1.permute_S || (a->ffn_parts && a->ln1.dy != a->d_x1)) return MMDA_EINVAL;
+  for (int i = 0; i < 3; ++i)
+    if (a->lnp[i].dy != a->d_orig + (int64_t)i * a->B * a->hs || a->lnp[i].permute_S) return MMDA_EINVAL;
   FusedBwdA P = *a;
   P.dbg = g_fr_dbg;
   hipLaunchKernelGGL(fused_bwd_a_kernel, dim3(ceil_div(a->B, a->nb)), dim3(FR_THREADS), 0, (hipStream_t)stream, P);
diff --git a/mmda_amd/csrc/rowlocal.h b/mmda_amd/csrc/rowlocal.h
--- a/mmda_amd/csrc/rowlocal.h
+++ b/mmda_amd/csrc/rowlocal.h
@@ -10,7 +10,8 @@
 }
 
 template <int NQ>
-__device__ __forceinline__ void ln_bwd_row(const mmda_ln_bwd_args& a, int row, int lane, float (&dg)[NQ], float (&db)[NQ]) {
+__device__ __forceinline__ void ln_bwd_row(const mmda_ln_bwd_args& a, int row, int lane, float (&dg)[NQ], float (&db)[NQ],
+                                           const float* lds_dy = nullptr, float* lds_dres = nullptr) {
   const int n = a.n;
   const float mean = a.mean[row], rstd = a.rstd[row];
   const int64_t drow = perm_row(row, a.permute_S, a.permute_B);
@@ -24,7 +25,7 @@
       int64_t idx = (int64_t)row * n + i;
       float x = act_fwd_p(a.act, a.x[idx], a.actp, (uint64_t)idx);
       if (a.res) x += a.res[idx] * drop_mul(a.drop_p, a.drop_seed, a.drop_site, (uint64_t)idx);
-      float dy = a.dy[drow * n + i];
+      float dy = lds_dy ? lds_dy[i] : a.dy[drow * n + i];
       xh[q] = (x - mean) * rstd;
       gdy[q] = dy * a.gamma[i];
       dg[q] += dy * xh[q];
@@ -48,7 +49,11 @@
         a.d_x[idx] = a.accumulate_dx ? a.d_x[idx] + d : d;
         if (a.act == MMDA_ACT_PRELU && z <= 0.f) dslope += dxp * z;
       }
-      if (a.d_res) a.d_res[idx] = dxp * drop_mul(a.drop_p, a.drop_seed, a.drop_site, (uint64_t)idx);
+      if (a.d_res) {
+        const float dr = dxp * drop_mul(a.drop_p, a.drop_seed, a.drop_site, (uint64_t)idx);
+        a.d_res[idx] = dr;
+        if (lds_dres) lds_dres[i] = dr;
+      }
     }
   }
   if (a.act == MMDA_ACT_PRELU && a.d_x && a.actp.dslope) {
@@ -58,7 +63,8 @@
 }
 
 template <int NQ>
-__device__ __forceinline__ void ln_fwd_row(const mmda_ln_args& a, int row, int lane) {
+__device__ __forceinline__ void ln_fwd_row(const mmda_ln_args& a, int row, int lane, const float* lds_x = nullptr,
+                                           const float* lds_res = nullptr, float* lds_y = nullptr) {
   const int n = a.n;
   float v[NQ];
   float s = 0.f;
@@ -68,8 +74,8 @@
     float x = 0.f;
     if (i < n) {
       int64_t idx = (int64_t)row * n + i;
-      x = act_fwd_p(a.act, a.x[idx], a.actp, (uint64_t)idx);
-      if (a.res) x += a.res[idx] * drop_mul(a.drop_p, a.drop_seed, a.drop_site, (uint64_t)idx);
+      x = act_fwd_p(a.act, lds_x ? lds_x[i] : a.x[idx], a.actp, (uint64_t)idx);
+      if (a.res) x += (lds_res ? lds_res[i] : a.res[idx]) * drop_mul(a.drop_p, a.drop_seed, a.drop_site, (uint64_t)idx);
     }
     v[q] = x;
     s += x;
@@ -93,7 +99,7 @@
   for (int q = 0; q < NQ; ++q) {
     int i = lane + 64 * q;
     float y = 0.f;
-    if (i < n) { y = (v[q] - mean) * rstd * a.gamma[i] + a.beta[i]; if (a.y) a.y[orow * n + i] = y; }
+    if (i < n) { y = (v[q] - mean) * rstd * a.gamma[i] + a.beta[i]; if (a.y) a.y[orow * n + i] = y; if (lds_y) lds_y[i] = y; }
     if (a.y_bf16 && i < a.ld_bf16) reinterpret_cast<unsigned short*>(a.y_bf16)[orow * a.ld_bf16 + i] = f2bf(y);
   }
 }
@@ -101,14 +107,15 @@
 constexpr int S6K = 6;
 
 __device__ __forceinline__ void attn_fwd_hd64_one(const float* __restrict__ qkv, int B, float* ctx, float* probs, float p, uint64_t seed,
-                                                  int site, int nhead, int bh, int d) {
+                                                  int site, int nhead, int bh, int d, const float* lds_qkv = nullptr, int lds_qkv_tok = 0,
+                                                  float* lds_ctx = nullptr, int lds_ctx_tok = 0) {
   constexpr int S = S6K, hd = 64;
   const int E = hd * nhead;
   const int b = bh / nhead, h = bh % nhead;
   float q[S], k[S], v[S];
 #pragma unroll
   for (int s = 0; s < S; ++s) {
-    const float* row = qkv + ((int64_t)s * B + b) * 3 * E + h * hd + d;
+    const float* row = lds_qkv ? lds_qkv + s * lds_qkv_tok + h * hd + d : qkv + ((int64_t)s * B + b) * 3 * E + h * hd + d;
     q[s] = row[0]; k[s] = row[E]; v[s] = row[2 * E];
   }
   const float scale = 1.0f / sqrtf((float)hd);
@@ -140,12 +147,15 @@
 #pragma unroll
     for (int j = 0; j < S; ++j) acc += pr[s][j] * v[j];
     ctx[((int64_t)s * B + b) * E + h * hd + d] = acc;
+    if (lds_ctx) lds_ctx[s * lds_ctx_tok + h * hd + d] = acc;
   }
 }
 
 
 __device__ __forceinline__ void attn_bwd_hd64_one(const float* __restrict__ qkv, const float* __restrict__ probs, const float* __restrict__ dctx,
-                                                  int B, float* dqkv, float p, uint64_t seed, int site, int nhead, int bh, int d) {
+                                                  int B, float* dqkv, float p, uint64_t seed, int site, int nhead, int bh, int d,
+                                                  const float* lds_dctx = nullptr, int lds_dctx_tok = 0, float* lds_dqkv = nullptr,
+                                                  int lds_dqkv_tok = 0) {
   constexpr int S = S6K, hd = 64;
   const int E = hd * nhead;
   const int b = bh / nhead, h = bh % nhead;
@@ -154,7 +164,7 @@
   for (int s = 0; s < S; ++s) {
     const float* row = qkv + ((int64_t)s * B + b) * 3 * E + h * hd + d;
     q[s] = row[0]; k[s] = row[E]; v[s] = row[2 * E];
-    dc[s] = dctx[((int64_t)s * B + b) * E + h * hd + d];
+    dc[s] = lds_dctx ? lds_dctx[s * lds_dctx_tok + h * hd + d] : dctx[((int64_t)s * B + b) * E + h * hd + d];
   }
   float P[S][S], Pd[S][S], dS[S][S];
 #pragma unroll
@@ -187,7 +197,11 @@
     }
     float* row = dqkv + ((int64_t)s * B + b) * 3 * E + h * hd + d;
     row[0] = dq * scale; row[E] = dk * scale; row[2 * E] = dv;
-  }
-}
-
-}
+    if (lds_dqkv) {
+      float* lrow = lds_dqkv + s * lds_dqkv_tok + h * hd + d;
+      lrow[0] = dq * scale; lrow[E] = dk * scale; lrow[2 * E] = dv;
+    }
+  }
+}
+
+}
```

Result: faster. 53890 samples/s, median of 6 (+1.1%).
